# ameli/gaussian-process-param-estimation

Hardware: AMD Instinct MI355X
Metric: log-likelihood evals/sec (N=16384 dense Matern-3/2) (higher is better)
Workload: dtype f64

## Files before the change

### gaussian-process-param-estimation_amd/csrc/gpmi_band.h

```cpp
#pragma once

#include "gpmi_internal.h"
#include "gpmi_band_plan.h"

namespace gpmi {

enum { KFAST = 0, KSLOW = 1 };

constexpr int HH_WAVES = 8;
constexpr int HH_THREADS = 64 * HH_WAVES;
constexpr int HH_RPW = 16;
constexpr int HH_ROWS = HH_WAVES * HH_RPW;
constexpr int HH_MAXG = 256;
constexpr int HH_PANEL_MAXG = 128;
constexpr int HH_PANEL_LDS = 96 * 1024;
constexpr int HH_PART_LD = 136;
constexpr int QT_ROWS = 64;
constexpr int TN_CH = 128;
constexpr int BAND_ULD = 384;
constexpr int LA_FREE = 32;
constexpr int LA_FREE_LATE = 64;
constexpr int LA_LATE_MT = 60;
constexpr int BAND_MAX_NPAD = HH_MAXG * HH_ROWS;

__global__ void hh_col_kernel(double* P, int64_t lda, int m, int c, double* part, double* pivrow,
                              double* tau);
__global__ void hh_panel_kernel(double* P, int64_t lda, int m, double* part, double* pivrow,
                                unsigned* counter, double* tau, int* err, unsigned spin_limit,
                                const int* guard, double* Uv, int64_t ldu);
__global__ void vcopy_kernel(const double* P, int64_t lda, int m, double* U, int64_t ldu);
__global__ void tn_partial_kernel(const double* P1, int64_t ld1, const double* P2, int64_t ld2,
                                  int m, double* part, const int* only_if);
__global__ void tn_reduce_kernel(const double* part, int nch, double* out, double scale,
                                 const int* only_if);
__global__ void tbuild_kernel(const double* VtV, const double* tau, double* T, const int* only_if);
__global__ void t_fallback_kernel(const double* V, int64_t ldv, int m, const double* tau,
                                  double* VtV, double* T, const int* only_if);
__global__ void symm_kernel(const double* A, int64_t lda, const double* U, int64_t ldu, int tr0,
                            int mt, int chunk, double* Xp);
__global__ void psum_kernel(const double* Xp, int nch, double* X);
__global__ void xt_q_kernel(const double* X, const double* T, double* X2);
__global__ void tn_partial_q_kernel(const double* P1, int64_t ld1, const double* P2, int64_t ld2,
                                    int m, double* part);
__global__ void z_q_kernel(const double* T, const double* M, double* Zh);
__global__ void w_q_kernel(const double* X, double* U, int64_t ldu, const double* Zh);
__global__ void syr2k_col_q_kernel(double* A, int64_t lda, const double* U, int64_t ldu, int tr0,
                                   const double* Ksrc);
__global__ void syr2k_kernel(double* A, int64_t lda, const double* U, int64_t ldu, int tr0,
                             int mt);
__global__ void syr2k_rest_kernel(double* A, int64_t lda, const double* U, int64_t ldu, int tr0,
                                  int mt, const uint32_t* order);
__global__ void syr2k_pipe_kernel(double* A, int64_t lda, const double* U, int64_t ldu, int tr0,
                                  int mt, int* cnt, int nmain, int filler, const double* Ksrc);
__global__ void bcr_f0_kernel(const double* Ab, int64_t lda, double* F0);
__global__ void bcr_chol_kernel(const double* Ab, int64_t lda, const double* etas, int lvl,
                                int first, const double* Din, int64_t sD, const double* Yin,
                                int64_t sY, double* Lout, int64_t sL, int lout, double* Zall,
                                int64_t sZ, double* logd, double* gpart, int* failv, int nt,
                                int64_t n);
__global__ void bcr_w_kernel(const double* Lin, int64_t sL, const double* Fin, int64_t sF,
                             double* W, int64_t sW, int m, int lvl, const double* dDin,
                             int64_t sdD, double* scr, double* dL);
__global__ void bcr_upd_kernel(const double* Ab, int64_t lda, const double* etas, int lvl,
                               const double* Din, int64_t sD, const double* Yin, int64_t sY,
                               const double* W, int64_t sW, const double* Zall, int64_t sZ,
                               double* Dout, double* Fout, double* Yout, int64_t sO, int64_t sOY,
                               int m, const double* L, const double* dL, int64_t sL,
                               const double* Fin, int64_t sF, const double* dFin, int64_t sdF,
                               double* dW);
__global__ void bcr_sinv_pre_kernel(const double* L, const double* dL, int64_t sL, const double* W,
                                    const double* dW, int64_t sW, double* X, double* dX,
                                    int64_t sX, double* Zd, double* dZd, int64_t sZd,
                                    double* trpart, double* dtrpart, int nt, int nlev, int64_t n,
                                    int ntan);
// ... 84 lines not shown
```

### gaussian-process-param-estimation_amd/csrc/gpmi_band.hip

```cpp

#include <hip/hip_runtime.h>
#include <math.h>
#include <stdint.h>

#include "gpmi_internal.h"
#include "gpmi_device.h"
#include "gpmi_lds_chol.h"
#include "gpmi_band.h"
#include "gpmi_tile.h"

#ifndef GPMI_BAND_STAMPS
#define GPMI_BAND_STAMPS 0
#endif

namespace gpmi {

__global__ __launch_bounds__(HH_THREADS) void hh_col_kernel(double* __restrict__ P, int64_t lda,
                                                      int m, int c, double* __restrict__ part,
                                                      double* __restrict__ pivrow,
                                                      double* __restrict__ tau) {
  __shared__ double sacc[HH_WAVES][HH_PART_LD];
  const int G = gridDim.x, g = blockIdx.x, t = threadIdx.x, lane = t & 63, w = t >> 6;
  const int j0 = lane, j1 = lane + 64;
  const int rbase = g * HH_ROWS + w * HH_RPW;
  double p0[HH_RPW], p1[HH_RPW];
#pragma unroll
// ... 366 lines not shown

__global__ __launch_bounds__(256) void t_fallback_kernel(const double* __restrict__ V,
                                                         int64_t ldv, int m,
                                                         const double* __restrict__ tau,
                                                         double* __restrict__ VtV,
                                                         double* __restrict__ T,
                                                         const int* __restrict__ only_if) {
  __shared__ double Ls[TS * DL];
  __shared__ double Aux[TS * RLD];
  __shared__ double stau[TS];
  static_assert(4 * GSTAGE <= TS * DL, "t_fallback_kernel: staging exceeds Ls");
  if (*only_if == 0) return;
  d4 acc[4][4];
  zero_tile(acc);
  for (int i0 = 0; i0 < m; i0 += TN_CH)
    gemm_tile<KSLOW, KSLOW, false>(V + (int64_t)i0 * ldv, ldv, V + (int64_t)i0 * ldv, ldv,
                                   min(TN_CH, m - i0), Ls, acc);
  store_tile(VtV, TS, acc, 1.0);
  __threadfence_block();
  __syncthreads();
  tbuild_body(VtV, tau, T, Ls, Aux, stau);
}

__global__ __launch_bounds__(256, 2) void symm_kernel(const double* __restrict__ A, int64_t lda,
                                                      const double* __restrict__ U, int64_t ldu,
                                                      int tr0, int mt, int chunk,
                                                      double* __restrict__ Xp) {
  __shared__ double smem[4 * GSTAGE];
  const int il = blockIdx.x, ch = blockIdx.y, nch = gridDim.y;
  const int I = tr0 + il;
  const int jl0 = ch * chunk, jl1 = min(mt, (ch + 1) * chunk);
  const int jsplit = min(jl1, max(jl0, il + 1));
  d4 acc[4][4];
  zero_tile(acc);
  for (int jl = jl0; jl < jsplit; ++jl) {
    const int J = tr0 + jl;
    gemm_tile<KFAST, KSLOW, false>(A + (int64_t)I * TS * lda + (int64_t)J * TS, lda,
                                   U + (int64_t)J * TS * ldu + TS, ldu, TS, smem, acc);
  }
  for (int jl = jsplit; jl < jl1; ++jl) {
    const int J = tr0 + jl;
    gemm_tile<KSLOW, KSLOW, false>(A + (int64_t)J * TS * lda + (int64_t)I * TS, lda,
                                   U + (int64_t)J * TS * ldu + TS, ldu, TS, smem, acc);
  }
  store_tile(Xp + ((int64_t)il * nch + ch) * TS * TS, TS, acc, 1.0);
}

__global__ __launch_bounds__(256) void psum_kernel(const double* __restrict__ Xp, int nch,
                                                   double* __restrict__ X) {
  const int il = blockIdx.y;
  const int e = (blockIdx.x * 256 + threadIdx.x) * 2;
  d2 s = {0.0, 0.0};
  for (int c0 = 0; c0 < nch; c0 += 8) {
    d2 x[8];
#pragma unroll
    for (int q = 0; q < 8; ++q)
      x[q] = c0 + q < nch
                 ? *reinterpret_cast<const d2*>(Xp + ((int64_t)il * nch + c0 + q) * TS * TS + e)
                 : d2{0.0, 0.0};
#pragma unroll
    for (int q = 0; q < 8; ++q)
      if (c0 + q < nch) s += x[q];
  }
  *reinterpret_cast<d2*>(X + (int64_t)il * TS * TS + e) = s;
}

__global__ __launch_bounds__(256, 2) void xt_q_kernel(const double* __restrict__ X,
                                                      const double* __restrict__ T,
                                                      double* __restrict__ X2) {
// ... 41 lines not shown
  d4 acc[2][2];
  load_quad(X + (int64_t)il * TS * TS, TS, acc, q >> 1, q & 1);
  gemm_quad2<KFAST, KSLOW, true, TS>(Ui + TS, ldu, Zh, TS, smem, acc, q >> 1, q & 1);
  store_quad(Ui, ldu, acc, 1.0, q >> 1, q & 1);
  store_quad(Ui + 2 * TS, ldu, acc, 1.0, q >> 1, q & 1);
}

__global__ __launch_bounds__(256, 2) void syr2k_col_q_kernel(double* __restrict__ A, int64_t lda,
                                                             const double* __restrict__ U,
                                                             int64_t ldu, int tr0,
                                                             const double* __restrict__ Ksrc) {
  __shared__ double smem[Q2_SMEM];
  const int I = tr0 + blockIdx.x, q = blockIdx.y;
  const int64_t off = (int64_t)I * TS * lda + (int64_t)tr0 * TS;
  double* C = A + off;
  d4 acc[2][2];
  load_quad((Ksrc ? Ksrc : A) + off, lda, acc, q >> 1, q & 1);
  gemm_quad2<KFAST, KFAST, true, 2 * TS>(U + (int64_t)I * TS * ldu, ldu,
                                         U + (int64_t)tr0 * TS * ldu + TS, ldu, smem, acc,
                                         q >> 1, q & 1);
  store_quad(C, lda, acc, 1.0, q >> 1, q & 1);
}

__device__ __forceinline__ void syr2k_tile(double* __restrict__ A, int64_t lda,
                                           const double* __restrict__ U, int64_t ldu, int I, int J,
                                           double* smem) {
  double* C = A + (int64_t)I * TS * lda + (int64_t)J * TS;
  d4 acc[4][4];
  load_tile(C, lda, acc);
  gemm_tile<KFAST, KFAST, true>(U + (int64_t)I * TS * ldu, ldu, U + (int64_t)J * TS * ldu + TS,
                                ldu, 2 * TS, smem, acc);
  store_tile(C, lda, acc, 1.0);
}

__global__ __launch_bounds__(256, 2) void syr2k_kernel(double* __restrict__ A, int64_t lda,
                                                       const double* __restrict__ U,
                                                       int64_t ldu, int tr0, int mt) {
  __shared__ double smem[4 * GSTAGE];
  int i, j;
  tri_decode(xcd_remap(blockIdx.x, gridDim.x), mt, &i, &j);
  syr2k_tile(A, lda, U, ldu, tr0 + i, tr0 + j, smem);
}

__global__ __launch_bounds__(256, 2) void syr2k_rest_kernel(double* __restrict__ A, int64_t lda,
                                                            const double* __restrict__ U,
                                                            int64_t ldu, int tr0, int mt,
                                                            const uint32_t* __restrict__ order) {
  __shared__ double smem[4 * GSTAGE];
  const int ntiles = (mt - 1) * mt / 2;
  if (order && gridDim.x >= 8) {
    const int nwg = gridDim.x, x = blockIdx.x & 7, l = blockIdx.x >> 3;
    const int nx = (nwg >> 3) + (x < (nwg & 7) ? 1 : 0);
    const int c0 = (int)((int64_t)ntiles * x / 8), c1 = (int)((int64_t)ntiles * (x + 1) / 8);
    for (int q = c0 + l; q < c1; q += nx) {
      const uint32_t o = order[q];
      syr2k_tile(A, lda, U, ldu, tr0 + 1 + (int)(o >> 16), tr0 + 1 + (int)(o & 0xffffu), smem);
    }
    return;
  }
  for (int q = blockIdx.x; q < ntiles; q += gridDim.x) {
    int i, j;
    tri_decode(q, mt - 1, &i, &j);
    syr2k_tile(A, lda, U, ldu, tr0 + i + 1, tr0 + j + 1, smem);
  }
}

__global__ __launch_bounds__(256, 1) void syr2k_pipe_kernel(double* __restrict__ A, int64_t lda,
                                                            const double* __restrict__ U,
                                                            int64_t ldu, int tr0, int mt,
                                                            int* __restrict__ cnt, int nmain,
                                                            int filler,
                                                            const double* __restrict__ Ksrc) {
  __shared__ double smem[4 * GSTAGE + 2];
  int* stk = reinterpret_cast<int*>(smem + 4 * GSTAGE);
  constexpr int KD = 2 * TS;
  constexpr int NS = KD / BK;
  constexpr int PER = (64 + NS - 1) / NS;
  const int ntiles = (mt - 1) * mt / 2;
  const int t = threadIdx.x, lane = t & 63, w = t >> 6;
  int q = blockIdx.x, qn = q + gridDim.x;
  if (cnt) {
    if (t == 0) {
      const int a = filler ? nmain + atomicAdd(cnt, 1) : q;
      stk[1] = a;
      stk[0] = a < ntiles ? nmain + atomicAdd(cnt, 1) : ntiles;
    }
    __syncthreads();
    q = stk[1];
    qn = stk[0];
// ... 2 lines not shown
  if (q >= ntiles) return;
  const int wr = w >> 1, wc = w & 1, fr = lane & 15, fk = lane >> 4;
  double* sA = smem;
  double* sB = smem + 2 * GSTAGE;
  auto tile_ptrs = [&](int qq, double** C, const double** P1, const double** P2) {
    int i, j;
    tri_decode(qq, mt - 1, &i, &j);
    const int I = tr0 + 1 + i, J = tr0 + 1 + j;
    *C = A + (int64_t)I * TS * lda + (int64_t)J * TS;
    *P1 = U + (int64_t)I * TS * ldu;
    *P2 = U + (int64_t)J * TS * ldu + TS;
  };
  const int64_t coff = (int64_t)(wr * 64 + fk) * lda + wc * 64 + fr;
  auto cidx = [&](int e) -> int64_t {
    return (int64_t)((e >> 4) * 16 + 4 * (e & 3)) * lda + ((e >> 2) & 3) * 16;
  };
  auto csrc = [&](const double* c) -> const double* { return Ksrc ? Ksrc + (c - A) : c; };
  d4 acc[4][4], cn[4][4], po[4][4];
  double* Cq;
  const double *P1, *P2;
  tile_ptrs(q, &Cq, &P1, &P2);
  load_tile(csrc(Cq), lda, acc);
  d2 ra[4], rb[4];
  gl_op<KFAST>(P1, ldu, 0, ra);
  gl_op<KFAST>(P2, ldu, 0, rb);
  st_op<KFAST>(sA, ra);
  st_op<KFAST>(sB, rb);
  __syncthreads();
  double* Cp = nullptr;
  bool has_p = false;
  int tk = 0;
  while (true) {
    const bool has_n = qn < ntiles;
    double* Cn = nullptr;
    const double *N1 = nullptr, *N2 = nullptr;
    if (has_n) tile_ptrs(qn, &Cn, &N1, &N2);
    const double* Cns = has_n ? csrc(Cn) : nullptr;
#pragma unroll
    for (int s = 0; s < NS; ++s) {
      const int cur = s & 1;
      const double* cA = sA + cur * GSTAGE;
      const double* cB = sB + cur * GSTAGE;
      const bool ld = s + 1 < NS || has_n;
      if (cnt && t == 0 && has_n) {
        if (s == NS / 2) tk = atomicAdd(cnt, 1);
        if (s == NS - 1) stk[0] = nmain + tk;
      }
      if (s + 1 < NS) {
        gl_op<KFAST>(P1, ldu, (s + 1) * BK, ra);
        gl_op<KFAST>(P2, ldu, (s + 1) * BK, rb);
      } else if (has_n) {
        gl_op<KFAST>(N1, ldu, 0, ra);
        gl_op<KFAST>(N2, ldu, 0, rb);
// ... 29 lines not shown
        st_op<KFAST>(sB + (cur ^ 1) * GSTAGE, rb);
      }
      __syncthreads();
    }
#pragma unroll
    for (int a = 0; a < 4; ++a)
#pragma unroll
      for (int c = 0; c < 4; ++c) {
        po[a][c] = acc[a][c];
        acc[a][c] = cn[a][c];
      }
    Cp = Cq;
    has_p = true;
    if (!has_n) break;
    q = qn;
    qn = cnt ? stk[0] : q + gridDim.x;
    Cq = Cn;
    P1 = N1;
    P2 = N2;
  }
#pragma unroll
  for (int e = 0; e < 64; ++e) Cp[coff + cidx(e)] = po[e >> 4][(e >> 2) & 3][e & 3];
}

__global__ __launch_bounds__(256) void qt_partial_kernel(const double* __restrict__ P,
                                                         int64_t lda, int m,
                                                         const double* __restrict__ Y,
                                                         double* __restrict__ part) {
  __shared__ double sy[QT_ROWS * RLD];
  const int g = blockIdx.x, t = threadIdx.x;
  const int i0 = g * QT_ROWS, i1 = min(m, i0 + QT_ROWS);
  for (int e = t; e < QT_ROWS * RLD; e += 256)
    sy[e] = (i0 + e / RLD < i1) ? Y[(int64_t)i0 * RLD + e] : 0.0;
  __syncthreads();
  const int a = t & 127, h = t >> 7;
  double s[8] = {0.0, 0.0, 0.0, 0.0, 0.0, 0.0, 0.0, 0.0};
  for (int i = i0; i < i1; ++i) {
    const double v = (i > a) ? P[(int64_t)i * lda + a] : (i == a ? 1.0 : 0.0);
    const double* yr = sy + (i - i0) * RLD + 8 * h;
#pragma unroll
    for (int q = 0; q < 8; ++q) s[q] += v * yr[q];
  }
#pragma unroll
  for (int q = 0; q < 8; ++q) part[((int64_t)g * TS + a) * RLD + 8 * h + q] = s[q];
}

// ... 471 lines not shown
```

### gaussian-process-param-estimation_amd/csrc/gpmi_band_api.hip

```cpp

#include <hip/hip_runtime.h>

#include <algorithm>
#include <cstdio>
#include <cstdlib>
#include <cstring>
#include <memory>
#include <vector>

#include "gpmi_band_host.h"

using namespace gpmi;

namespace {

std::vector<double> pack_rhs(const gpmi_band* b, const double* rhs, int64_t ld, int nrhs) {
  std::vector<double> h((size_t)b->n_pad * RLD, 0.0);
  for (int64_t i = 0; i < b->n; ++i)
    for (int c = 0; c < nrhs; ++c) h[(size_t)i * RLD + c] = rhs[i * ld + c];
  return h;
}

}

// ... 10 lines not shown
  std::unique_ptr<gpmi_band> owner(new gpmi_band());
  gpmi_band* b = owner.get();
  BandReduce& r = b->red;
  b->device = v.device;
  b->n = v.n;
  b->n_pad = v.n_pad;
  b->nt = (int)(v.n_pad / TS);
  const int64_t np = b->n_pad;
  const int nt = b->nt;
  b->eval.plan = BandPlan(nt);
  b->eval.levels = bcr_levels(nt);
  HIP_TRY(hipDeviceGetAttribute(&b->ncu, hipDeviceAttributeMultiprocessorCount, v.device));
  const size_t nch = (size_t)std::max<int64_t>(1, (np + TN_CH - 1) / TN_CH);
  const size_t blk = (size_t)TS * TS;
  HIP_TRY(hipStreamCreateWithFlags(&b->stream.h, hipStreamNonBlocking));
  for (Event* ev : {&b->ev0, &b->ev1, &b->ev2, &b->ev3}) HIP_TRY(hipEventCreate(&ev->h));
  HIP_TRY(hipStreamCreateWithFlags(&b->side.h, hipStreamNonBlocking));
  if (const char* la = std::getenv("GPMI_BAND_LA")) r.lookahead = std::atoi(la);
  if (const char* po = std::getenv("GPMI_BAND_POISON")) r.poison = std::atoi(po) != 0;
  if (const char* v = std::getenv("GPMI_LA_FREE")) r.la_free = std::max(1, std::atoi(v));
  if (const char* v = std::getenv("GPMI_LA_FREE_LATE")) r.la_free_late = std::max(1, std::atoi(v));
  if (const char* v = std::getenv("GPMI_LA_LATE_MT")) r.la_late_mt = std::atoi(v);
  if (const char* pm = std::getenv("GPMI_BAND_PANEL")) r.panel_mode = std::strcmp(pm, "hh") == 0;
  if (const char* bm = std::getenv("GPMI_BAND_BCR"))
    b->eval.bcr_mode = std::max(0, std::min(2, std::atoi(bm)));
  if (const char* fo = std::getenv("GPMI_CQ_FO"))
    if (std::atoi(fo) == 0) r.cq_fo[1] = r.cq_fo[2] = 0.0;
  if (const char* sl = std::getenv("GPMI_CHASE_SPIN_LIMIT"))
    b->eig.chase_spin = (unsigned)std::strtoul(sl, nullptr, 10);
  if (const char* sl = std::getenv("GPMI_HH_SPIN_LIMIT"))
    r.spin_limit = (unsigned)std::strtoul(sl, nullptr, 10);

  if (r.lookahead) {
    int lo = 0, hi = 0;
    HIP_TRY(hipDeviceGetStreamPriorityRange(&lo, &hi));
    HIP_TRY(hipStreamCreateWithPriority(&r.s_pan.h, hipStreamNonBlocking, hi));
    for (Event* ev : {&r.ev_col, &r.ev_pan})
      HIP_TRY(hipEventCreateWithFlags(&ev->h, sync_event_flags()));
  }
  for (Event* ev : {&r.ev_q, &r.ev_v, &r.ev_t, &r.ev_rc})
    HIP_TRY(hipEventCreateWithFlags(&ev->h, sync_event_flags()));
  HIP_TRY(b->Ab.reserve(np * np));
  HIP_TRY(r.U.reserve(np * BAND_ULD));
  HIP_TRY(r.X.reserve(np * TS));
  HIP_TRY(r.X2.reserve(np * TS));
  HIP_TRY(r.Xp.reserve(xp_tiles(nt, b->ncu) * blk));
// ... 181 lines not shown
```

### gaussian-process-param-estimation_amd/csrc/gpmi_band_host.h

```cpp
#pragma once

#include <vector>

#include "gpmi_internal.h"
#include "gpmi_band.h"
#include "gpmi_band_plan.h"
#include "gpmi_host.h"
#include "../../include/gpmi.h"

static_assert(gpmi::BAND_TS == GPMI_TS && gpmi::BAND_RLD == GPMI_RHS_LD &&
                  gpmi::BAND_TAN_MAX == GPMI_BAND_TAN_MAX,
              "gpmi_band_plan.h restates these");

namespace gpmi {
int op_view(const gpmi_op* op, OpView* v);
}

#pragma GCC visibility push(hidden)

namespace gpmi {

constexpr int TS = GPMI_TS;
constexpr int RLD = GPMI_RHS_LD;
constexpr int OUT_LD = BAND_OUT_LD;
// ... 9 lines not shown
  DevBuf<double> part;
  DevBuf<double> pivrow;
  DevBuf<double> tau;
  DevBuf<double> Tm;
  DevBuf<double> tnp;
  DevBuf<double> tnp2;
  DevBuf<double> VtV, M, Zh;
  DevBuf<double> qtp;
  DevBuf<double> qa, qb;
  DevBuf<unsigned> ctr;
  DevBuf<int> err;
  int panel_maxg = HH_PANEL_MAXG;
  unsigned spin_limit = 1u << 24;
  int panel_fallbacks = 0;
  int panel_mode = 0;
  int cq_fallbacks = 0;
  DevBuf<double> Qb, cqpart, cqG;
  DevBuf<double> cqL;
  DevBuf<double> cqLinv;
  DevBuf<double> cqS;
  DevBuf<double> cqscr;
  DevBuf<int> cqflag;
  int la_free = LA_FREE, la_free_late = LA_FREE_LATE, la_late_mt = LA_LATE_MT;
  bool poison = false;
  int cq_panel_fallbacks = 0;
  int cq_host_checks = 0;
  DevBuf<uint32_t> rorder;
  std::vector<int64_t> rorder_off;
  DevBuf<double> cqMinv;
  DevBuf<double> cqUS;
  DevBuf<double> cqW;
  Event ev_rc;
  std::vector<char> t_from_q;
  std::vector<char> v_in_u;
  double cq_fo[3] = {0.0, 1e-4, 3e-8};
};

struct BandIo {
  int cap = 0;
  DevBuf<double> etas;
  DevBuf<double> out;
  DevBuf<int> info;
  hipError_t reserve(int neta) {
    const int c = BandPlan::io_capacity(neta);
    return regrow(&cap, c, {sized(etas, c), sized(out, (size_t)c * OUT_LD), sized(info, c)});
  }
// ... 116 lines not shown
```

### gaussian-process-param-estimation_amd/csrc/gpmi_band_reduce.hip

```cpp

#include <hip/hip_runtime.h>

#include <algorithm>
#include <chrono>
#include <cstdio>
#include <cstdlib>
#include <vector>

#include "gpmi_band_host.h"

using namespace gpmi;

namespace gpmi {

int qt_panel(gpmi_band* b, int j, hipStream_t st) {
  BandReduce& r = b->red;
  const int64_t np = b->n_pad;
  const int64_t r0 = (int64_t)(j + 1) * TS, c0 = (int64_t)j * TS;
  const int m = (int)(np - r0);
  const int G = (m + QT_ROWS - 1) / QT_ROWS;
  const double* P = b->Ab + r0 * np + c0;
  double* Yr = b->Y + r0 * RLD;
  hipLaunchKernelGGL(qt_partial_kernel, dim3(G), dim3(256), 0, st, P, np, m, Yr, r.qtp);
  LAUNCH_CHECK("qt_partial_kernel");
// ... 118 lines not shown
                         r.pivrow, tau);
      LAUNCH_CHECK("hh_col_kernel");
    }
  }
  return 0;
}

int band_reduce_pass(gpmi_band* b, const double* K, const std::vector<double>* yh, int mode) {
  BandReduce& r = b->red;
  hipStream_t s = b->stream;
  const int64_t np = b->n_pad;
  const int nt = b->nt;
  HIP_TRY(hipMemsetAsync(r.err, 0, 16, s));
  if (mode == 0) HIP_TRY(hipMemsetAsync(r.cqflag, 0, sizeof(int) * 8 * nt, s));
  HIP_TRY(hipEventRecord(b->ev0, s));
  const auto host_t0 = std::chrono::steady_clock::now();
  if (yh) {
    HIP_TRY(hipMemcpyAsync(b->Y, yh->data(), sizeof(double) * yh->size(), hipMemcpyHostToDevice,
                          b->side));
  }
  std::fill(r.t_from_q.begin(), r.t_from_q.end(), 0);
  std::fill(r.v_in_u.begin(), r.v_in_u.end(), 0);
  const bool la = mode != 2 && r.lookahead && r.s_pan;
  const bool k_first = mode == 0 && la && nt > 2;
  if (k_first && r.poison)
    HIP_TRY(hipMemsetAsync(b->Ab, 0xff, sizeof(double) * np * np, s));
  if (k_first)
    HIP_TRY(hipMemcpy2DAsync(b->Ab, sizeof(double) * np, K, sizeof(double) * np,
                            sizeof(double) * TS, np, hipMemcpyDeviceToDevice, s));
  else
    HIP_TRY(hipMemcpyAsync(b->Ab, K, sizeof(double) * np * np, hipMemcpyDeviceToDevice, s));
  bool ahead = false;
  for (int j = 0; j + 1 < nt; ++j) {
    const int64_t r0 = (int64_t)(j + 1) * TS, c0 = (int64_t)j * TS;
    const int m = (int)(np - r0), mt = nt - j - 1;
    double* P = b->Ab + r0 * np + c0;
    double* tau = r.tau + (int64_t)j * TS;
    double* T = r.Tm + (int64_t)j * TS * TS;
    if (!ahead) {
      int rc = panel_qr(b, j, s, mode);
      if (rc) return rc;
    }
    ahead = false;
    double* Ur = r.U + r0 * BAND_ULD;
    if (!r.v_in_u[j]) {
      hipLaunchKernelGGL(vcopy_kernel, dim3((unsigned)((int64_t)m * TS / 256)), dim3(256), 0, s,
// ... 6 lines not shown
    if (r.t_from_q[j]) {
      hipLaunchKernelGGL(t_fallback_kernel, dim3(1), dim3(256), 0, b->side, Ur + TS,
                         (int64_t)BAND_ULD, m, tau, r.VtV, T, r.cqflag + 8 * j + 4);
      LAUNCH_CHECK("t_fallback_kernel");
    } else {
      hipLaunchKernelGGL(tn_partial_kernel, dim3(nch), dim3(256), 0, b->side, Ur + TS,
                         (int64_t)BAND_ULD, Ur + TS, (int64_t)BAND_ULD, m, r.tnp2, nullptr);
      LAUNCH_CHECK("tn_partial_kernel");
      hipLaunchKernelGGL(tn_reduce_kernel, dim3(TS * TS / 64), dim3(256), 0, b->side, r.tnp2,
                         nch, r.VtV, 1.0, nullptr);
      LAUNCH_CHECK("tn_reduce_kernel");
      hipLaunchKernelGGL(tbuild_kernel, dim3(1), dim3(256), 0, b->side, r.VtV, tau, T, nullptr);
      LAUNCH_CHECK("tbuild_kernel");
    }
    r.t_from_q[j] = 0;
    HIP_TRY(hipEventRecord(r.ev_t, b->side));
    if (yh) {
      int rc = qt_panel(b, j, b->side);
      if (rc) return rc;
    }
    const int chunk = symm_chunk(mt, 2 * b->ncu);
    const int sch = (mt + chunk - 1) / chunk;
    const double* ksrc = (k_first && j == 0) ? K : nullptr;
    hipLaunchKernelGGL(symm_kernel, dim3(mt, sch), dim3(256), 0, s, ksrc ? ksrc : b->Ab, np,
                       r.U, (int64_t)BAND_ULD, j + 1, mt, chunk, r.Xp);
    LAUNCH_CHECK("symm_kernel");
    hipLaunchKernelGGL(psum_kernel, dim3(TS * TS / 512, mt), dim3(256), 0, s, r.Xp, sch, r.X);
    LAUNCH_CHECK("psum_kernel");
    HIP_TRY(hipStreamWaitEvent(s, r.ev_t, 0));
    hipLaunchKernelGGL(xt_q_kernel, dim3(mt, 4), dim3(256), 0, s, r.X, T, r.X2);
    LAUNCH_CHECK("xt_q_kernel");
    hipLaunchKernelGGL(tn_partial_q_kernel, dim3(nch, 4), dim3(256), 0, s, Ur + TS,
                       (int64_t)BAND_ULD, r.X2, (int64_t)TS, m, r.tnp);
    LAUNCH_CHECK("tn_partial_q_kernel");
    hipLaunchKernelGGL(tn_reduce_kernel, dim3(TS * TS / 64), dim3(256), 0, s, r.tnp, nch, r.M,
                       1.0, nullptr);
    LAUNCH_CHECK("tn_reduce_kernel");
    hipLaunchKernelGGL(z_q_kernel, dim3(4), dim3(256), 0, s, T, r.M, r.Zh);
    LAUNCH_CHECK("z_q_kernel");
    hipLaunchKernelGGL(w_q_kernel, dim3(mt, 4), dim3(256), 0, s, r.X2, Ur, (int64_t)BAND_ULD,
                       r.Zh);
    LAUNCH_CHECK("w_q_kernel");
    const int next_g = (int)((np - r0 - TS + HH_ROWS - 1) / HH_ROWS);
    if (la && j + 2 < nt && (mode == 0 || next_g <= r.panel_maxg)) {
      hipLaunchKernelGGL(syr2k_col_q_kernel, dim3(mt, 4), dim3(256), 0, s, b->Ab, np, r.U,
                         (int64_t)BAND_ULD, j + 1, ksrc);
      LAUNCH_CHECK("syr2k_col_q_kernel");
      HIP_TRY(hipEventRecord(r.ev_col, s));
      HIP_TRY(hipStreamWaitEvent(r.s_pan, r.ev_col, 0));
      const bool pipe = mode == 0;
      const int rest = (mt - 1) * mt / 2;
      const int la_free = mt < r.la_late_mt ? r.la_free_late : r.la_free;
      const int nmain = std::min(rest, std::max(1, b->ncu - la_free));
      int* tcnt = pipe ? r.cqflag + 8 * j + 6 : nullptr;
      if (pipe) {
        hipLaunchKernelGGL(syr2k_pipe_kernel, dim3(nmain), dim3(256), 0, r.s_pan, b->Ab, np,
                           r.U, (int64_t)BAND_ULD, j + 1, mt, tcnt, nmain, 0, ksrc);
        LAUNCH_CHECK("syr2k_pipe_kernel");
      } else {
        const int cap = r.la_grid > 0 ? r.la_grid : std::max(64, b->ncu - next_g);
        hipLaunchKernelGGL(syr2k_rest_kernel, dim3(std::min(rest, cap)), dim3(256), 0, r.s_pan,
                           b->Ab, np, r.U, (int64_t)BAND_ULD, j + 1,
                           mt, r.rorder ? r.rorder + r.rorder_off[mt - 1] : nullptr);
        LAUNCH_CHECK("syr2k_rest_kernel");
      }
      HIP_TRY(hipEventRecord(r.ev_pan, r.s_pan));
      bool guard = false;
      int rc = panel_qr(b, j + 1, s, mode, pipe ? &guard : nullptr);
      if (rc) return rc;
      if (tcnt && rest > nmain) {
        hipLaunchKernelGGL(syr2k_pipe_kernel, dim3(std::min(la_free, rest - nmain)), dim3(256),
                           0, s, b->Ab, np, r.U, (int64_t)BAND_ULD, j + 1, mt, tcnt, nmain, 1,
                           ksrc);
        LAUNCH_CHECK("syr2k_pipe_kernel");
      }
      HIP_TRY(hipStreamWaitEvent(s, r.ev_pan, 0));
      if (guard) {
        rc = cq_guard(b, j + 1, s);
        if (rc) return rc;
      }
      ahead = true;
    } else {
      const int tiles = mt * (mt + 1) / 2;
      hipLaunchKernelGGL(syr2k_kernel, dim3(tiles), dim3(256), 0, s, b->Ab, np, r.U,
                         (int64_t)BAND_ULD, j + 1, mt);
      LAUNCH_CHECK("syr2k_kernel");
    }
  }
  if (yh) {
    HIP_TRY(hipEventRecord(r.ev_q, b->side));
    HIP_TRY(hipStreamWaitEvent(s, r.ev_q, 0));
  }
  if (mode == 0 && nt > 1) {
    hipLaunchKernelGGL(cq_top_kernel, dim3(nt - 1), dim3(256), 0, s, r.cqL, r.cqLinv, r.cqflag,
                       r.cqS, r.cqscr, b->Ab, np);
    LAUNCH_CHECK("cq_top_kernel");
  }
  HIP_TRY(hipEventRecord(b->ev1, s));
  const double host_enqueue_ms =
      std::chrono::duration<double, std::milli>(std::chrono::steady_clock::now() - host_t0).count();
  int herr = 0;
  std::vector<int> hflag(mode == 0 ? 8 * nt : 0);
  HIP_TRY(hipMemcpyAsync(&herr, r.err, sizeof(int), hipMemcpyDeviceToHost, s));
  if (mode == 0)
    HIP_TRY(hipMemcpyAsync(hflag.data(), r.cqflag, sizeof(int) * hflag.size(),
                          hipMemcpyDeviceToHost, s));
  HIP_TRY(hipEventSynchronize(b->ev1));
  HIP_TRY(hipStreamSynchronize(s));
// ... 34 lines not shown
```

### gaussian-process-param-estimation_amd/csrc/gpmi_tile.h

```cpp
#pragma once

#include "gpmi_device.h"
#include "gpmi_band.h"

namespace gpmi {

constexpr int SLD = 144;
constexpr int GSTAGE = 16 * SLD;

template <int L>
__device__ __forceinline__ void gl_op(const double* __restrict__ base, int64_t ld, int k0,
                                      d2 (&r)[4]) {
  if (L == KFAST) {
    gload_slab(base, ld, k0, r);
    return;
  }
  const int t = threadIdx.x, kk = t >> 4, c0 = (t & 15) * 8;
  const double* p = base + (int64_t)(k0 + kk) * ld + c0;
#pragma unroll
  for (int q = 0; q < 4; ++q) r[q] = *reinterpret_cast<const d2*>(p + 2 * q);
}

template <int L>
__device__ __forceinline__ void st_op(double* s, const d2 (&r)[4]) {
  if (L == KFAST) {
    sstore_slab(s, r);
    return;
  }
  const int t = threadIdx.x, kk = t >> 4, c0 = (t & 15) * 8;
#pragma unroll
  for (int q = 0; q < 4; ++q) *reinterpret_cast<d2*>(s + kk * SLD + c0 + 2 * q) = r[q];
}

template <int L>
__device__ __forceinline__ double fr_op(const double* s, int row, int k) {
  return L == KFAST ? s[slab_off(row, k)] : s[k * SLD + row];
}

template <int AL, int BL, bool NEG>
__device__ __forceinline__ void gemm_tile(const double* __restrict__ P1, int64_t ld1,
                                          const double* __restrict__ P2, int64_t ld2, int kdim,
                                          double* smem, d4 (&acc)[4][4]) {
  const int t = threadIdx.x, lane = t & 63, w = t >> 6;
  const int wr = w >> 1, wc = w & 1, fr = lane & 15, fk = lane >> 4;
  double* sA = smem;
  double* sB = smem + 2 * GSTAGE;
  d2 ra[4], rb[4];
  gl_op<AL>(P1, ld1, 0, ra);
  gl_op<BL>(P2, ld2, 0, rb);
  st_op<AL>(sA, ra);
  st_op<BL>(sB, rb);
  __syncthreads();
  __builtin_amdgcn_s_waitcnt(0x0F70);
  const int nsteps = kdim / BK;
  for (int s = 0; s < nsteps; ++s) {
    const int cur = s & 1;
    const double* cA = sA + cur * GSTAGE;
    const double* cB = sB + cur * GSTAGE;
    if (s + 1 < nsteps) {
      gl_op<AL>(P1, ld1, (s + 1) * BK, ra);
      gl_op<BL>(P2, ld2, (s + 1) * BK, rb);
    }
#pragma unroll
    for (int kk = 0; kk < BK / 4; ++kk) {
      double a[4], b[4];
// ... 252 lines not shown
```

Baseline: 48.07.

## Add early-issue k-loop variant with buffer loads for band SYR2K/SYMM kernels

Templates the symm, syr2k, syr2k_rest and syr2k_pipe kernels on a k-loop mode and makes the new early mode the default. The early mode issues global loads two stages ahead through buffer resources with scalar-uniform pointers. It also interleaves C-tile load and store with the MFMA stages and pins the instruction schedule with sched_group_barriers. In symm, consecutive J tiles are merged into one long k-loop. The aim is to hide global-memory latency and cut per-tile prologue cost, at the price of more registers, more complex scheduling, and reliance on inline scheduling hints.

```diff
diff --git a/gaussian-process-param-estimation_amd/csrc/gpmi_band.h b/gaussian-process-param-estimation_amd/csrc/gpmi_band.h
--- a/gaussian-process-param-estimation_amd/csrc/gpmi_band.h
+++ b/gaussian-process-param-estimation_amd/csrc/gpmi_band.h
@@ -36,6 +36,7 @@
 __global__ void tbuild_kernel(const double* VtV, const double* tau, double* T, const int* only_if);
 __global__ void t_fallback_kernel(const double* V, int64_t ldv, int m, const double* tau,
                                   double* VtV, double* T, const int* only_if);
+template <int KL>
 __global__ void symm_kernel(const double* A, int64_t lda, const double* U, int64_t ldu, int tr0,
                             int mt, int chunk, double* Xp);
 __global__ void psum_kernel(const double* Xp, int nch, double* X);
@@ -46,10 +47,13 @@
 __global__ void w_q_kernel(const double* X, double* U, int64_t ldu, const double* Zh);
 __global__ void syr2k_col_q_kernel(double* A, int64_t lda, const double* U, int64_t ldu, int tr0,
                                    const double* Ksrc);
+template <int KL>
 __global__ void syr2k_kernel(double* A, int64_t lda, const double* U, int64_t ldu, int tr0,
                              int mt);
+template <int KL>
 __global__ void syr2k_rest_kernel(double* A, int64_t lda, const double* U, int64_t ldu, int tr0,
                                   int mt, const uint32_t* order);
+template <int KL>
 __global__ void syr2k_pipe_kernel(double* A, int64_t lda, const double* U, int64_t ldu, int tr0,
                                   int mt, int* cnt, int nmain, int filler, const double* Ksrc);
 __global__ void bcr_f0_kernel(const double* Ab, int64_t lda, double* F0);
diff --git a/gaussian-process-param-estimation_amd/csrc/gpmi_band.hip b/gaussian-process-param-estimation_amd/csrc/gpmi_band.hip
--- a/gaussian-process-param-estimation_amd/csrc/gpmi_band.hip
+++ b/gaussian-process-param-estimation_amd/csrc/gpmi_band.hip
@@ -2,6 +2,8 @@
 #include <hip/hip_runtime.h>
 #include <math.h>
 #include <stdint.h>
+
+#include <type_traits>
 
 #include "gpmi_internal.h"
 #include "gpmi_device.h"
@@ -414,6 +416,7 @@
   tbuild_body(VtV, tau, T, Ls, Aux, stau);
 }
 
+template <int KL>
 __global__ __launch_bounds__(256, 2) void symm_kernel(const double* __restrict__ A, int64_t lda,
                                                       const double* __restrict__ U, int64_t ldu,
                                                       int tr0, int mt, int chunk,
@@ -425,18 +428,38 @@
   const int jsplit = min(jl1, max(jl0, il + 1));
   d4 acc[4][4];
   zero_tile(acc);
-  for (int jl = jl0; jl < jsplit; ++jl) {
-    const int J = tr0 + jl;
-    gemm_tile<KFAST, KSLOW, false>(A + (int64_t)I * TS * lda + (int64_t)J * TS, lda,
-                                   U + (int64_t)J * TS * ldu + TS, ldu, TS, smem, acc);
-  }
-  for (int jl = jsplit; jl < jl1; ++jl) {
-    const int J = tr0 + jl;
-    gemm_tile<KSLOW, KSLOW, false>(A + (int64_t)J * TS * lda + (int64_t)I * TS, lda,
-                                   U + (int64_t)J * TS * ldu + TS, ldu, TS, smem, acc);
+  if constexpr (KL == KLOOP_LATE) {
+    for (int jl = jl0; jl < jsplit; ++jl) {
+      const int J = tr0 + jl;
+      gemm_tile<KFAST, KSLOW, false>(A + (int64_t)I * TS * lda + (int64_t)J * TS, lda,
+                                     U + (int64_t)J * TS * ldu + TS, ldu, TS, smem, acc);
+    }
+    for (int jl = jsplit; jl < jl1; ++jl) {
+      const int J = tr0 + jl;
+      gemm_tile<KSLOW, KSLOW, false>(A + (int64_t)J * TS * lda + (int64_t)I * TS, lda,
+                                     U + (int64_t)J * TS * ldu + TS, ldu, TS, smem, acc);
+    }
+    store_tile(Xp + ((int64_t)il * nch + ch) * TS * TS, TS, acc, 1.0);
+    return;
+  }
+  if (jsplit > jl0) {
+    const int J = tr0 + jl0;
+    gemm_tile<KFAST, KSLOW, false, KL>(A + (int64_t)I * TS * lda + (int64_t)J * TS, lda,
+                                       U + (int64_t)J * TS * ldu + TS, ldu, (jsplit - jl0) * TS,
+                                       smem, acc);
+  }
+  if (jl1 > jsplit) {
+    const int J = tr0 + jsplit;
+    gemm_tile<KSLOW, KSLOW, false, KL>(A + (int64_t)J * TS * lda + (int64_t)I * TS, lda,
+                                       U + (int64_t)J * TS * ldu + TS, ldu, (jl1 - jsplit) * TS,
+                                       smem, acc);
   }
   store_tile(Xp + ((int64_t)il * nch + ch) * TS * TS, TS, acc, 1.0);
 }
+template __global__ void symm_kernel<KLOOP_LATE>(const double*, int64_t, const double*, int64_t,
+                                                 int, int, int, double*);
+template __global__ void symm_kernel<KLOOP_EARLY>(const double*, int64_t, const double*, int64_t,
+                                                  int, int, int, double*);
 
 __global__ __launch_bounds__(256) void psum_kernel(const double* __restrict__ Xp, int nch,
                                                    double* __restrict__ X) {
@@ -524,49 +547,155 @@
   store_quad(C, lda, acc, 1.0, q >> 1, q & 1);
 }
 
+template <int KL>
 __device__ __forceinline__ void syr2k_tile(double* __restrict__ A, int64_t lda,
                                            const double* __restrict__ U, int64_t ldu, int I, int J,
                                            double* smem) {
   double* C = A + (int64_t)I * TS * lda + (int64_t)J * TS;
   d4 acc[4][4];
   load_tile(C, lda, acc);
-  gemm_tile<KFAST, KFAST, true>(U + (int64_t)I * TS * ldu, ldu, U + (int64_t)J * TS * ldu + TS,
-                                ldu, 2 * TS, smem, acc);
+  gemm_tile<KFAST, KFAST, true, KL>(U + (int64_t)I * TS * ldu, ldu,
+                                    U + (int64_t)J * TS * ldu + TS, ldu, 2 * TS, smem, acc);
   store_tile(C, lda, acc, 1.0);
 }
 
+template <int KL>
 __global__ __launch_bounds__(256, 2) void syr2k_kernel(double* __restrict__ A, int64_t lda,
                                                        const double* __restrict__ U,
                                                        int64_t ldu, int tr0, int mt) {
   __shared__ double smem[4 * GSTAGE];
   int i, j;
   tri_decode(xcd_remap(blockIdx.x, gridDim.x), mt, &i, &j);
-  syr2k_tile(A, lda, U, ldu, tr0 + i, tr0 + j, smem);
-}
-
+  syr2k_tile<KL>(A, lda, U, ldu, tr0 + i, tr0 + j, smem);
+}
+template __global__ void syr2k_kernel<KLOOP_LATE>(double*, int64_t, const double*, int64_t, int,
+                                                  int);
+template __global__ void syr2k_kernel<KLOOP_EARLY>(double*, int64_t, const double*, int64_t, int,
+                                                   int);
+
+template <int KL>
 __global__ __launch_bounds__(256, 2) void syr2k_rest_kernel(double* __restrict__ A, int64_t lda,
                                                             const double* __restrict__ U,
                                                             int64_t ldu, int tr0, int mt,
                                                             const uint32_t* __restrict__ order) {
   __shared__ double smem[4 * GSTAGE];
   const int ntiles = (mt - 1) * mt / 2;
-  if (order && gridDim.x >= 8) {
+  const bool grouped = order && gridDim.x >= 8;
+  int q = blockIdx.x, q1 = ntiles, step = gridDim.x;
+  if (grouped) {
     const int nwg = gridDim.x, x = blockIdx.x & 7, l = blockIdx.x >> 3;
-    const int nx = (nwg >> 3) + (x < (nwg & 7) ? 1 : 0);
-    const int c0 = (int)((int64_t)ntiles * x / 8), c1 = (int)((int64_t)ntiles * (x + 1) / 8);
-    for (int q = c0 + l; q < c1; q += nx) {
+    step = (nwg >> 3) + (x < (nwg & 7) ? 1 : 0);
+    q = (int)((int64_t)ntiles * x / 8) + l;
+    q1 = (int)((int64_t)ntiles * (x + 1) / 8);
+  }
+  for (; q < q1; q += step) {
+    int i, j;
+    if (grouped) {
       const uint32_t o = order[q];
-      syr2k_tile(A, lda, U, ldu, tr0 + 1 + (int)(o >> 16), tr0 + 1 + (int)(o & 0xffffu), smem);
-    }
-    return;
-  }
-  for (int q = blockIdx.x; q < ntiles; q += gridDim.x) {
-    int i, j;
-    tri_decode(q, mt - 1, &i, &j);
-    syr2k_tile(A, lda, U, ldu, tr0 + i + 1, tr0 + j + 1, smem);
-  }
-}
-
+      i = (int)(o >> 16);
+      j = (int)(o & 0xffffu);
+    } else {
+      tri_decode(q, mt - 1, &i, &j);
+    }
+    i = __builtin_amdgcn_readfirstlane(i);
+    j = __builtin_amdgcn_readfirstlane(j);
+    int64_t ldc = lda;
+    asm volatile("" : "+s"(ldc));
+    syr2k_tile<KL>(A, ldc, U, ldu, tr0 + 1 + i, tr0 + 1 + j, smem);
+  }
+}
+template __global__ void syr2k_rest_kernel<KLOOP_LATE>(double*, int64_t, const double*, int64_t,
+                                                       int, int, const uint32_t*);
+template __global__ void syr2k_rest_kernel<KLOOP_EARLY>(double*, int64_t, const double*, int64_t,
+                                                        int, int, const uint32_t*);
+
+
+template <int S, int N, class F>
+__device__ __forceinline__ void static_for(F& f) {
+  if constexpr (S < N) {
+    f(std::integral_constant<int, S>{});
+    static_for<S + 1, N>(f);
+  }
+}
+
+template <int S>
+__device__ __forceinline__ void syr2k_pipe_stage_early(
+    __amdgpu_buffer_rsrc_t R1, __amdgpu_buffer_rsrc_t R2, int64_t ldu, uint32_t vo, int k2,
+    bool has2, double* sA, double* sB, d4 (&acc)[4][4], d2 (&ra)[4], d2 (&rb)[4], double (&a)[4],
+    double (&b)[4], const double* __restrict__ Cld, double* __restrict__ Cst, bool has_p,
+    int64_t lda, d4 (&cn)[4][4], d4 (&po)[4][4]) {
+  constexpr int CUR = S & 1;
+  constexpr int PER = 4;
+  const int t = threadIdx.x, lane = t & 63, w = t >> 6;
+  const int wr = w >> 1, wc = w & 1, fr = lane & 15, fk = lane >> 4;
+  const double* cA = sA + CUR * GSTAGE;
+  const double* cB = sB + CUR * GSTAGE;
+  double* nA = sA + (CUR ^ 1) * GSTAGE;
+  double* nB = sB + (CUR ^ 1) * GSTAGE;
+  auto cidx = [&](int e) -> int64_t {
+    return (int64_t)((e >> 4) * 16 + 4 * (e & 3)) * lda + ((e >> 2) & 3) * 16;
+  };
+  sstore_slab(nA, ra);
+  sstore_slab(nB, rb);
+#pragma unroll
+  for (int kk = 0; kk < BK / 4; ++kk) {
+    double an[4], bn[4];
+#pragma unroll
+    for (int i = 0; i < 4; ++i) {
+      if (kk == 0 && i == 1) {
+        pin_behind_mfma<0x200, 4, 2>();
+        if (has2) {
+          gload_slab_u(R1, ldu, k2, vo, ra);
+          gload_slab_u(R2, ldu, k2, vo, rb);
+        }
+        if (has_p) {
+#pragma unroll
+          for (int u = 0; u < PER; ++u) {
+            const int e = S * PER + u;
+            Cst[cidx(e)] = po[e >> 4][(e >> 2) & 3][e & 3];
+          }
+        }
+#pragma unroll
+        for (int u = 0; u < PER; ++u) {
+          const int e = S * PER + u;
+          cn[e >> 4][(e >> 2) & 3][e & 3] = Cld[cidx(e)];
+        }
+      }
+      if ((kk == 0 && i == 1) || (kk > 0 && i == 0)) {
+        const double* fA = kk + 1 < BK / 4 ? cA : nA;
+        const double* fB = kk + 1 < BK / 4 ? cB : nB;
+        const int kn = ((kk + 1) * 4) % BK + fk;
+#pragma unroll
+        for (int ii = 0; ii < 4; ++ii) an[ii] = fA[slab_off(wr * 64 + ii * 16 + fr, kn)];
+#pragma unroll
+        for (int j = 0; j < 4; ++j) bn[j] = fB[slab_off(wc * 64 + j * 16 + fr, kn)];
+      }
+#pragma unroll
+      for (int j = 0; j < 4; ++j) acc[i][j] = mfma64_neg(a[i], b[j], acc[i][j]);
+    }
+#pragma unroll
+    for (int i = 0; i < 4; ++i) {
+      a[i] = an[i];
+      b[i] = bn[i];
+    }
+    if (kk == 1) {
+      pin_behind_mfma<0x20, 4, 1>();
+      pin_behind_mfma<0x100, 4, 1>();
+      __builtin_amdgcn_sched_group_barrier(0x8, 4, 0);
+      pin_kstep<0>();
+      __builtin_amdgcn_sched_barrier(0);
+      __syncthreads();
+      __builtin_amdgcn_sched_barrier(0);
+    }
+  }
+  pin_kstep<8>();
+  pin_kstep<0>();
+  __builtin_amdgcn_sched_barrier(0);
+  __syncthreads();
+  __builtin_amdgcn_sched_barrier(0);
+}
+
+template <int KL>
 __global__ __launch_bounds__(256, 1) void syr2k_pipe_kernel(double* __restrict__ A, int64_t lda,
                                                             const double* __restrict__ U,
                                                             int64_t ldu, int tr0, int mt,
@@ -615,13 +744,80 @@
   tile_ptrs(q, &Cq, &P1, &P2);
   load_tile(csrc(Cq), lda, acc);
   d2 ra[4], rb[4];
+  double* Cp = nullptr;
+  bool has_p = false;
+  if constexpr (KL == KLOOP_EARLY) {
+    static_assert(NS % 2 == 0 && PER == 4, "syr2k_pipe_kernel: stage pairs, 4 C values a stage");
+    const uint32_t vo = slab_voff(ldu);
+    {
+      const __amdgpu_buffer_rsrc_t R1 = slab_rsrc(uniform_ptr(P1)),
+                                   R2 = slab_rsrc(uniform_ptr(P2));
+      gload_slab_u(R1, ldu, 0, vo, ra);
+      gload_slab_u(R2, ldu, 0, vo, rb);
+      sstore_slab(sA, ra);
+      sstore_slab(sB, rb);
+      __builtin_amdgcn_s_waitcnt(0x0F70);
+      gload_slab_u(R1, ldu, BK, vo, ra);
+      gload_slab_u(R2, ldu, BK, vo, rb);
+    }
+    __syncthreads();
+    double a[4], b[4];
+#pragma unroll
+    for (int i = 0; i < 4; ++i) a[i] = sA[slab_off(wr * 64 + i * 16 + fr, fk)];
+#pragma unroll
+    for (int j = 0; j < 4; ++j) b[j] = sB[slab_off(wc * 64 + j * 16 + fr, fk)];
+    __builtin_amdgcn_sched_barrier(0);
+    int tk = 0;
+    while (true) {
+      const bool has_n = qn < ntiles;
+      double* Cn = Cq;
+      const double *N1 = P1, *N2 = P2;
+      if (has_n) tile_ptrs(qn, &Cn, &N1, &N2);
+      const __amdgpu_buffer_rsrc_t R1 = slab_rsrc(uniform_ptr(P1)),
+                                   R2 = slab_rsrc(uniform_ptr(P2)),
+                                   RN1 = slab_rsrc(uniform_ptr(N1)),
+                                   RN2 = slab_rsrc(uniform_ptr(N2));
+      const double* Cld = csrc(Cn) + coff;
+      double* Cst = has_p ? Cp + coff : nullptr;
+      auto stage = [&](auto sc) {
+        constexpr int s = decltype(sc)::value;
+        if (cnt && t == 0 && has_n) {
+          if (s == NS / 2) tk = atomicAdd(cnt, 1);
+          if (s == NS - 1) stk[0] = nmain + tk;
+        }
+        if constexpr (s + 2 < NS)
+          syr2k_pipe_stage_early<s>(R1, R2, ldu, vo, (s + 2) * BK, true, sA, sB, acc, ra, rb, a,
+                                    b, Cld, Cst, has_p, lda, cn, po);
+        else
+          syr2k_pipe_stage_early<s>(RN1, RN2, ldu, vo, (s + 2 - NS) * BK, has_n, sA, sB, acc, ra,
+                                    rb, a, b, Cld, Cst, has_p, lda, cn, po);
+      };
+      static_for<0, NS>(stage);
+#pragma unroll
+      for (int a4 = 0; a4 < 4; ++a4)
+#pragma unroll
+        for (int c = 0; c < 4; ++c) {
+          po[a4][c] = acc[a4][c];
+          acc[a4][c] = cn[a4][c];
+        }
+      Cp = Cq;
+      has_p = true;
+      if (!has_n) break;
+      q = qn;
+      qn = cnt ? stk[0] : q + gridDim.x;
+      Cq = Cn;
+      P1 = N1;
+      P2 = N2;
+    }
+#pragma unroll
+    for (int e = 0; e < 64; ++e) Cp[coff + cidx(e)] = po[e >> 4][(e >> 2) & 3][e & 3];
+    return;
+  }
   gl_op<KFAST>(P1, ldu, 0, ra);
   gl_op<KFAST>(P2, ldu, 0, rb);
   st_op<KFAST>(sA, ra);
   st_op<KFAST>(sB, rb);
   __syncthreads();
-  double* Cp = nullptr;
-  bool has_p = false;
   int tk = 0;
   while (true) {
     const bool has_n = qn < ntiles;
@@ -697,6 +893,10 @@
 #pragma unroll
   for (int e = 0; e < 64; ++e) Cp[coff + cidx(e)] = po[e >> 4][(e >> 2) & 3][e & 3];
 }
+template __global__ void syr2k_pipe_kernel<KLOOP_LATE>(double*, int64_t, const double*, int64_t,
+                                                       int, int, int*, int, int, const double*);
+template __global__ void syr2k_pipe_kernel<KLOOP_EARLY>(double*, int64_t, const double*, int64_t,
+                                                        int, int, int*, int, int, const double*);
 
 __global__ __launch_bounds__(256) void qt_partial_kernel(const double* __restrict__ P,
                                                          int64_t lda, int m,
diff --git a/gaussian-process-param-estimation_amd/csrc/gpmi_band_api.hip b/gaussian-process-param-estimation_amd/csrc/gpmi_band_api.hip
--- a/gaussian-process-param-estimation_amd/csrc/gpmi_band_api.hip
+++ b/gaussian-process-param-estimation_amd/csrc/gpmi_band_api.hip
@@ -56,6 +56,11 @@
   if (const char* v = std::getenv("GPMI_LA_FREE_LATE")) r.la_free_late = std::max(1, std::atoi(v));
   if (const char* v = std::getenv("GPMI_LA_LATE_MT")) r.la_late_mt = std::atoi(v);
   if (const char* pm = std::getenv("GPMI_BAND_PANEL")) r.panel_mode = std::strcmp(pm, "hh") == 0;
+  if (const char* m = std::getenv("GPMI_BAND_KLOOP")) {
+    if (!std::strcmp(m, "early")) r.kloop = KLOOP_EARLY;
+    else if (!std::strcmp(m, "late")) r.kloop = KLOOP_LATE;
+    else return set_errorf(-1009, "GPMI_BAND_KLOOP must be early or late (got %s)", m);
+  }
   if (const char* bm = std::getenv("GPMI_BAND_BCR"))
     b->eval.bcr_mode = std::max(0, std::min(2, std::atoi(bm)));
   if (const char* fo = std::getenv("GPMI_CQ_FO"))
diff --git a/gaussian-process-param-estimation_amd/csrc/gpmi_band_host.h b/gaussian-process-param-estimation_amd/csrc/gpmi_band_host.h
--- a/gaussian-process-param-estimation_amd/csrc/gpmi_band_host.h
+++ b/gaussian-process-param-estimation_amd/csrc/gpmi_band_host.h
@@ -55,6 +55,7 @@
   DevBuf<double> cqscr;
   DevBuf<int> cqflag;
   int la_free = LA_FREE, la_free_late = LA_FREE_LATE, la_late_mt = LA_LATE_MT;
+  int kloop = KLOOP_EARLY;
   bool poison = false;
   int cq_panel_fallbacks = 0;
   int cq_host_checks = 0;
diff --git a/gaussian-process-param-estimation_amd/csrc/gpmi_band_reduce.hip b/gaussian-process-param-estimation_amd/csrc/gpmi_band_reduce.hip
--- a/gaussian-process-param-estimation_amd/csrc/gpmi_band_reduce.hip
+++ b/gaussian-process-param-estimation_amd/csrc/gpmi_band_reduce.hip
@@ -164,6 +164,8 @@
   std::fill(r.t_from_q.begin(), r.t_from_q.end(), 0);
   std::fill(r.v_in_u.begin(), r.v_in_u.end(), 0);
   const bool la = mode != 2 && r.lookahead && r.s_pan;
+  const bool early = r.kloop == KLOOP_EARLY;
+  const auto pipe_kernel = early ? syr2k_pipe_kernel<KLOOP_EARLY> : syr2k_pipe_kernel<KLOOP_LATE>;
   const bool k_first = mode == 0 && la && nt > 2;
   if (k_first && r.poison)
     HIP_TRY(hipMemsetAsync(b->Ab, 0xff, sizeof(double) * np * np, s));
@@ -216,8 +218,9 @@
     const int chunk = symm_chunk(mt, 2 * b->ncu);
     const int sch = (mt + chunk - 1) / chunk;
     const double* ksrc = (k_first && j == 0) ? K : nullptr;
-    hipLaunchKernelGGL(symm_kernel, dim3(mt, sch), dim3(256), 0, s, ksrc ? ksrc : b->Ab, np,
-                       r.U, (int64_t)BAND_ULD, j + 1, mt, chunk, r.Xp);
+    hipLaunchKernelGGL(early ? symm_kernel<KLOOP_EARLY> : symm_kernel<KLOOP_LATE>, dim3(mt, sch),
+                       dim3(256), 0, s, ksrc ? ksrc : b->Ab, np, r.U, (int64_t)BAND_ULD, j + 1,
+                       mt, chunk, r.Xp);
     LAUNCH_CHECK("symm_kernel");
     hipLaunchKernelGGL(psum_kernel, dim3(TS * TS / 512, mt), dim3(256), 0, s, r.Xp, sch, r.X);
     LAUNCH_CHECK("psum_kernel");
@@ -248,14 +251,15 @@
       const int nmain = std::min(rest, std::max(1, b->ncu - la_free));
       int* tcnt = pipe ? r.cqflag + 8 * j + 6 : nullptr;
       if (pipe) {
-        hipLaunchKernelGGL(syr2k_pipe_kernel, dim3(nmain), dim3(256), 0, r.s_pan, b->Ab, np,
+        hipLaunchKernelGGL(pipe_kernel, dim3(nmain), dim3(256), 0, r.s_pan, b->Ab, np,
                            r.U, (int64_t)BAND_ULD, j + 1, mt, tcnt, nmain, 0, ksrc);
         LAUNCH_CHECK("syr2k_pipe_kernel");
       } else {
         const int cap = r.la_grid > 0 ? r.la_grid : std::max(64, b->ncu - next_g);
-        hipLaunchKernelGGL(syr2k_rest_kernel, dim3(std::min(rest, cap)), dim3(256), 0, r.s_pan,
-                           b->Ab, np, r.U, (int64_t)BAND_ULD, j + 1,
-                           mt, r.rorder ? r.rorder + r.rorder_off[mt - 1] : nullptr);
+        hipLaunchKernelGGL(early ? syr2k_rest_kernel<KLOOP_EARLY> : syr2k_rest_kernel<KLOOP_LATE>,
+                           dim3(std::min(rest, cap)), dim3(256), 0, r.s_pan, b->Ab, np, r.U,
+                           (int64_t)BAND_ULD, j + 1, mt,
+                           r.rorder ? r.rorder + r.rorder_off[mt - 1] : nullptr);
         LAUNCH_CHECK("syr2k_rest_kernel");
       }
       HIP_TRY(hipEventRecord(r.ev_pan, r.s_pan));
@@ -263,7 +267,7 @@
       int rc = panel_qr(b, j + 1, s, mode, pipe ? &guard : nullptr);
       if (rc) return rc;
       if (tcnt && rest > nmain) {
-        hipLaunchKernelGGL(syr2k_pipe_kernel, dim3(std::min(la_free, rest - nmain)), dim3(256),
+        hipLaunchKernelGGL(pipe_kernel, dim3(std::min(la_free, rest - nmain)), dim3(256),
                            0, s, b->Ab, np, r.U, (int64_t)BAND_ULD, j + 1, mt, tcnt, nmain, 1,
                            ksrc);
         LAUNCH_CHECK("syr2k_pipe_kernel");
@@ -276,8 +280,9 @@
       ahead = true;
     } else {
       const int tiles = mt * (mt + 1) / 2;
-      hipLaunchKernelGGL(syr2k_kernel, dim3(tiles), dim3(256), 0, s, b->Ab, np, r.U,
-                         (int64_t)BAND_ULD, j + 1, mt);
+      hipLaunchKernelGGL(early ? syr2k_kernel<KLOOP_EARLY> : syr2k_kernel<KLOOP_LATE>,
+                         dim3(tiles), dim3(256), 0, s, b->Ab, np, r.U, (int64_t)BAND_ULD, j + 1,
+                         mt);
       LAUNCH_CHECK("syr2k_kernel");
     }
   }
diff --git a/gaussian-process-param-estimation_amd/csrc/gpmi_tile.h b/gaussian-process-param-estimation_amd/csrc/gpmi_tile.h
--- a/gaussian-process-param-estimation_amd/csrc/gpmi_tile.h
+++ b/gaussian-process-param-estimation_amd/csrc/gpmi_tile.h
@@ -37,10 +37,144 @@
   return L == KFAST ? s[slab_off(row, k)] : s[k * SLD + row];
 }
 
+__device__ __forceinline__ const double* uniform_ptr(const double* p) {
+  const uint64_t v = reinterpret_cast<uint64_t>(p);
+  const uint32_t lo = __builtin_amdgcn_readfirstlane((uint32_t)v);
+  const uint32_t hi = __builtin_amdgcn_readfirstlane((uint32_t)(v >> 32));
+  return reinterpret_cast<const double*>(((uint64_t)hi << 32) | lo);
+}
+
+template <int L>
+__device__ __forceinline__ uint32_t op_voff(int64_t ld) {
+  if (L == KFAST) return slab_voff(ld);
+  const int t = threadIdx.x;
+  return (uint32_t)(((t >> 4) * ld + (t & 15) * 8) * 8);
+}
+
+template <int L>
+__device__ __forceinline__ void gl_op_u(const double* __restrict__ base, int64_t ld, int k0,
+                                        uint32_t voff, d2 (&r)[4]) {
+  if (L == KFAST) {
+    gload_slab_u(slab_rsrc(base), ld, k0, voff, r);
+    return;
+  }
+  const __amdgpu_buffer_rsrc_t rs = slab_rsrc(base + (int64_t)k0 * ld);
+#pragma unroll
+  for (int q = 0; q < 4; ++q)
+    r[q] = __builtin_bit_cast(d2, __builtin_amdgcn_raw_buffer_load_b128(rs, voff, 16 * q, 0));
+}
+
+template <int AL, int BL, bool NEG, int CUR>
+__device__ __forceinline__ void gemm_tile_early_stage(const double* P1, int64_t ld1,
+                                                      const double* P2, int64_t ld2,
+                                                      uint32_t vo1, uint32_t vo2, int s, bool has2,
+                                                      double* sA, double* sB, d4 (&acc)[4][4],
+                                                      d2 (&ra)[4], d2 (&rb)[4], double (&a)[4],
+                                                      double (&b)[4]) {
+  const int t = threadIdx.x, lane = t & 63, w = t >> 6;
+  const int wr = w >> 1, wc = w & 1, fr = lane & 15, fk = lane >> 4;
+  const double* cA = sA + CUR * GSTAGE;
+  const double* cB = sB + CUR * GSTAGE;
+  double* nA = sA + (CUR ^ 1) * GSTAGE;
+  double* nB = sB + (CUR ^ 1) * GSTAGE;
+  st_op<AL>(nA, ra);
+  st_op<BL>(nB, rb);
+#pragma unroll
+  for (int kk = 0; kk < BK / 4; ++kk) {
+    double an[4], bn[4];
+#pragma unroll
+    for (int i = 0; i < 4; ++i) {
+      if (kk == 0 && i == 1) {
+        pin_behind_mfma<0x200, 4, 2>();
+        if (has2) {
+          gl_op_u<AL>(P1, ld1, (s + 2) * BK, vo1, ra);
+          gl_op_u<BL>(P2, ld2, (s + 2) * BK, vo2, rb);
+        }
+      }
+      if ((kk == 0 && i == 1) || (kk > 0 && i == 0)) {
+        const double* fA = kk + 1 < BK / 4 ? cA : nA;
+        const double* fB = kk + 1 < BK / 4 ? cB : nB;
+        const int kn = ((kk + 1) * 4) % BK + fk;
+#pragma unroll
+        for (int ii = 0; ii < 4; ++ii) an[ii] = fr_op<AL>(fA, wr * 64 + ii * 16 + fr, kn);
+#pragma unroll
+        for (int j = 0; j < 4; ++j) bn[j] = fr_op<BL>(fB, wc * 64 + j * 16 + fr, kn);
+      }
+#pragma unroll
+      for (int j = 0; j < 4; ++j)
+        acc[i][j] = NEG ? mfma64_neg(a[i], b[j], acc[i][j]) : mfma64(a[i], b[j], acc[i][j]);
+    }
+#pragma unroll
+    for (int i = 0; i < 4; ++i) {
+      a[i] = an[i];
+      b[i] = bn[i];
+    }
+    if (kk == 1) {
+      __builtin_amdgcn_sched_group_barrier(0x8, 4, 0);
+      pin_behind_mfma<0x100, 4, 1>();
+      __builtin_amdgcn_sched_group_barrier(0x8, 4, 0);
+      pin_kstep<0>();
+      __builtin_amdgcn_sched_barrier(0);
+      __syncthreads();
+      __builtin_amdgcn_sched_barrier(0);
+    }
+  }
+  pin_kstep<8>();
+  pin_kstep<0>();
+  __builtin_amdgcn_sched_barrier(0);
+  __syncthreads();
+  __builtin_amdgcn_sched_barrier(0);
+}
+
 template <int AL, int BL, bool NEG>
+__device__ __forceinline__ void gemm_tile_early(const double* __restrict__ P1, int64_t ld1,
+                                                const double* __restrict__ P2, int64_t ld2,
+                                                int kdim, double* smem, d4 (&acc)[4][4]) {
+  const int t = threadIdx.x, lane = t & 63, w = t >> 6;
+  const int wr = w >> 1, wc = w & 1, fr = lane & 15, fk = lane >> 4;
+  double* sA = smem;
+  double* sB = smem + 2 * GSTAGE;
+  const int nsteps = kdim / BK;
+  const uint32_t vo1 = op_voff<AL>(ld1), vo2 = op_voff<BL>(ld2);
+  d2 ra[4], rb[4];
+  gl_op_u<AL>(P1, ld1, 0, vo1, ra);
+  gl_op_u<BL>(P2, ld2, 0, vo2, rb);
+  st_op<AL>(sA, ra);
+  st_op<BL>(sB, rb);
+  __builtin_amdgcn_s_waitcnt(0x0F70);
+  gl_op_u<AL>(P1, ld1, BK, vo1, ra);
+  gl_op_u<BL>(P2, ld2, BK, vo2, rb);
+  __syncthreads();
+  double a[4], b[4];
+#pragma unroll
+  for (int i = 0; i < 4; ++i) a[i] = fr_op<AL>(sA, wr * 64 + i * 16 + fr, fk);
+#pragma unroll
+  for (int j = 0; j < 4; ++j) b[j] = fr_op<BL>(sB, wc * 64 + j * 16 + fr, fk);
+  __builtin_amdgcn_sched_barrier(0);
+  for (int s = 0; s < nsteps; s += 2) {
+    gemm_tile_early_stage<AL, BL, NEG, 0>(P1, ld1, P2, ld2, vo1, vo2, s, s + 2 < nsteps, sA, sB,
+                                          acc, ra, rb, a, b);
+    gemm_tile_early_stage<AL, BL, NEG, 1>(P1, ld1, P2, ld2, vo1, vo2, s + 1, s + 3 < nsteps, sA,
+                                          sB, acc, ra, rb, a, b);
+  }
+}
+
+template <int AL, int BL, bool NEG, int KL = KLOOP_LATE>
 __device__ __forceinline__ void gemm_tile(const double* __restrict__ P1, int64_t ld1,
                                           const double* __restrict__ P2, int64_t ld2, int kdim,
                                           double* smem, d4 (&acc)[4][4]) {
+  if constexpr (KL == KLOOP_EARLY) {
+    P1 = uniform_ptr(P1);
+    P2 = uniform_ptr(P2);
+    if constexpr (AL == KFAST && BL == KFAST) {
+      d4 racc[2];
+      tile_mma<false, NEG, KLOOP_EARLY>(P1, ld1, P2, ld2, kdim, smem, smem + 2 * GSTAGE, acc,
+                                        nullptr, racc);
+    } else {
+      gemm_tile_early<AL, BL, NEG>(P1, ld1, P2, ld2, kdim, smem, acc);
+    }
+    return;
+  }
   const int t = threadIdx.x, lane = t & 63, w = t >> 6;
   const int wr = w >> 1, wc = w & 1, fr = lane & 15, fk = lane >> 4;
   double* sA = smem;
```

After: 48.12 (median of 6 runs). About the same (+0.1%).
